# criteo/tf-yarn

Measured on AMD Instinct MI355X. Metric: examples/sec (whole node), Criteo wide-and-deep, higher is better.
Workload: dtype bf16; 1 GPU; model=wide_and_deep_criteo, global_batch=65536, per_gpu_batch=65536, dense_features=13, sparse_features=26, embedding_dim=16, table_rows_per_feature=1000000, parallelism=dp1, alltoall_mode=unprobed

## Files before the change

tf_yarn_amd/ops/__init__.py:

```python

from __future__ import annotations

import functools
import logging
import math
import os
from typing import NamedTuple, Optional, Tuple

import torch

logger = logging.getLogger(__name__)

try:
    from tf_yarn_amd.ops import _C
    HAVE_EXT = True
except ImportError as _e:
    _C = None
    HAVE_EXT = False
    _IMPORT_ERROR = _e


def _require_ext() -> None:
    if not HAVE_EXT:
        raise RuntimeError(
# ... 913 lines not shown
            batch, n_features * dim, device=table.device,
            dtype=torch.bfloat16 if out_bf16 else torch.float32)
        col_offset = 0
    if (out.dim() != 2 or out.shape[0] != batch or col_offset < 0
            or col_offset + n_features * dim > out.shape[1]):
        raise ValueError(
            f"the [{batch}, {n_features * dim}] block at column "
            f"{col_offset} does not fit out {tuple(out.shape)}")
    if _on_gpu(table, ids, out):
        _require_ext()
        bag_scale, flat = _C.emb_bag_fwd(table, ids, bag_offsets,
                                         n_features, offsets, weights,
                                         combiner, out, col_offset)
        return out, bag_scale, flat
    if _bounds_debug():
        _debug_check_bags(bag_offsets, ids.numel())
    bag_scale, flat = _emb_bag_fwd_ref(table, ids, bag_offsets, n_features,
                                       offsets, weights, combiner, out,
                                       col_offset)
    return out, bag_scale, flat


def emb_bag_bwd_rows(grad_out: torch.Tensor, bag_offsets: torch.Tensor,
                     bag_scale: torch.Tensor, dim: int, n_features: int, *,
                     weights: Optional[torch.Tensor] = None,
                     col_offset: int = 0,
                     nnz: Optional[int] = None) -> torch.Tensor:
    if nnz is None and weights is not None:
        nnz = int(weights.numel())
    batch = _check_bags(None, bag_offsets, n_features, weights, nnz)
    if bag_scale.numel() != batch * n_features:
        raise ValueError("bag_scale must have one entry per bag")
    if (grad_out.dim() != 2 or grad_out.shape[0] != batch or col_offset < 0
            or col_offset + n_features * dim > grad_out.shape[1]):
        raise ValueError(
            f"the [{batch}, {n_features * dim}] block at column "
            f"{col_offset} does not fit grad_out {tuple(grad_out.shape)}")
    if _on_gpu(grad_out, bag_offsets, bag_scale):
        _require_ext()
        if nnz is None:
            nnz = int(bag_offsets[-1].item())
        if grad_out.stride(1) != 1 or grad_out.stride(0) < grad_out.shape[1]:
            grad_out = grad_out.contiguous()
        return _C.emb_bag_bwd_rows(grad_out, bag_offsets, bag_scale, dim,
                                   n_features, nnz, weights, col_offset)
    _, lens = _bag_lengths(bag_offsets)
    n_bags = batch * n_features
    if _bounds_debug():
        _debug_check_bags(bag_offsets, int(lens.sum().item()))
    bag = torch.repeat_interleave(torch.arange(n_bags), lens)
    s = bag_scale[bag]
    if weights is not None:
        s = s * weights
    g = grad_out[:, col_offset:col_offset + n_features * dim] \
        .reshape(n_bags, dim)[bag]
    return (g.float() * s.unsqueeze(1)).to(grad_out.dtype)


class EmbeddingBagFn(torch.autograd.Function):

    @staticmethod
    def forward(ctx, table, ids, bag_offsets, n_features, offsets, weights,
                combiner, out_bf16, sink, dense, col_offset, wrap):
        dim = table.shape[1]
        batch = (bag_offsets.numel() - 1) // n_features
        out = None
        if dense is not None or col_offset:
            out = torch.empty(
                batch, col_offset + n_features * dim, device=table.device,
                dtype=torch.bfloat16 if out_bf16 else torch.float32)
            n_dense = 0
            if dense is not None:
                n_dense = dense.shape[1]
                out[:, :n_dense] = dense.to(out.dtype)
            out[:, n_dense:col_offset] = 0
        out, bag_scale, flat_ids = emb_bag_fwd(
            table.detach(), ids, bag_offsets, n_features, offsets=offsets,
            weights=weights, combiner=combiner, out=out,
            col_offset=col_offset, out_bf16=out_bf16)
        ctx.sink, ctx.wrap = sink, wrap
        ctx.dims = (dim, n_features, col_offset, ids.numel())
        ctx.weights = weights
        ctx.save_for_backward(bag_offsets, bag_scale, flat_ids)
        return out

    @staticmethod
    def backward(ctx, grad_out):
        bag_offsets, bag_scale, flat_ids = ctx.saved_tensors
        dim, n_features, col_offset, nnz = ctx.dims
        rows = emb_bag_bwd_rows(grad_out, bag_offsets, bag_scale, dim,
                                n_features, weights=ctx.weights,
                                col_offset=col_offset, nnz=nnz)
        ctx.sink.append(ctx.wrap((flat_ids, rows)))
        return (None,) * 12


def col_reduce_dot(x: torch.Tensor, dy: torch.Tensor) -> torch.Tensor:
    if _on_gpu(x, dy):
        _require_ext()
        return _C.col_reduce_dot(x.contiguous(), dy.contiguous())
    return (x.float() * dy.float().unsqueeze(1)).sum(dim=0)


def fused_head_grads_enabled() -> bool:
    return _env_switch_on("MIYARN_FUSED_HEAD_GRADS")


def col_reduce_dot_sum(x: torch.Tensor, dy: torch.Tensor,
                       out_dtype: torch.dtype = torch.float32):
    if _on_gpu(x, dy):
        _require_ext()
        if out_dtype in (torch.float32, torch.bfloat16):
            dw, db = _C.col_reduce_dot_sum(x.contiguous(), dy.contiguous(),
                                           out_dtype == torch.bfloat16)
            return dw, db
        dw, db = _C.col_reduce_dot_sum(x.contiguous(), dy.contiguous(),
                                       False)
        return dw.to(out_dtype), db.to(out_dtype)
    dw = (x.float() * dy.float().unsqueeze(1)).sum(dim=0)
    db = dy.float().sum().reshape(1)
    return dw.to(out_dtype), db.to(out_dtype)


def row_dot(x: torch.Tensor, w: torch.Tensor,
            bias: "torch.Tensor | None" = None) -> torch.Tensor:
    if _on_gpu(x, w) and x.size(1) % 4 == 0 and x.size(1) <= 512:
        _require_ext()
        return _C.row_dot(x.contiguous(), w.contiguous(), bias)
    y = x @ w
    return y if bias is None else y + bias


def gemm_bt(a: torch.Tensor, b: torch.Tensor,
            bias: "torch.Tensor | None" = None,
            relu: bool = False) -> torch.Tensor:
    if _on_gpu(a, b):
        _require_ext()
        return _C.gemm_bt(a.contiguous(), b.contiguous(), bias, relu)
    out = a.float() @ b.float().t()
    if bias is not None:
        out = out + bias.float()
    if relu:
        out = torch.relu(out)
    return out.to(a.dtype)


class ScalarHeadFn(torch.autograd.Function):

    @staticmethod
    def forward(ctx, x, weight, bias):
        ctx.save_for_backward(x, weight)
        if _on_gpu(x, weight) and x.size(1) % 4 == 0 \
                and x.size(1) <= 512 and bias.numel() == 1:
            _require_ext()
            return _C.row_dot(x.contiguous(), weight.contiguous(),
                              bias.reshape(1))
        return x @ weight + bias

    @staticmethod
    def backward(ctx, dy):
        x, weight = ctx.saved_tensors
        dy = dy.contiguous()
        dx = dw = db = None
        if ctx.needs_input_grad[0]:
            dx = dy.unsqueeze(1) * weight.unsqueeze(0)
        if ctx.needs_input_grad[1] and ctx.needs_input_grad[2] \
                and _on_gpu(x, dy) and x.dtype == dy.dtype \
                and fused_head_grads_enabled():
            dw, db = col_reduce_dot_sum(x, dy, weight.dtype)
            return dx, dw, db
        if ctx.needs_input_grad[1]:
            dw = col_reduce_dot(x, dy).to(weight.dtype)
        if ctx.needs_input_grad[2]:
            db = dy.sum().reshape(1).to(weight.dtype)
        return dx, dw, db


class BCEHeadFn(torch.autograd.Function):

    @staticmethod
    def forward(ctx, deep, wide, dhead, labels):
        if deep.is_cuda and HAVE_EXT and deep.dtype == torch.bfloat16 \
                and wide.dtype == torch.bfloat16 \
                and dhead.dtype == torch.bfloat16:
            loss, sig = _C.bce_head_fwd(
                deep.contiguous(), wide.contiguous(), dhead.contiguous(),
                labels.contiguous().float())
        else:
            z = (deep.float() + wide.float() + dhead.float())
            labels = labels.float()
            loss = torch.nn.functional.binary_cross_entropy_with_logits(
                z, labels, reduction="none")
            sig = torch.sigmoid(z).to(deep.dtype)
        ctx.save_for_backward(sig, labels)
        ctx.dtype = deep.dtype
        return loss

    @staticmethod
    def backward(ctx, g):
        sig, labels = ctx.saved_tensors
        if sig.is_cuda and HAVE_EXT and sig.dtype == torch.bfloat16:
            dl = _C.bce_head_bwd(sig, labels.contiguous().float(),
                                 g.contiguous().float())
        else:
            dl = ((sig.float() - labels.float()) * g.float()).to(ctx.dtype)
        return dl, dl, dl, None


def bce_head_loss(deep: torch.Tensor, wide: torch.Tensor,
                  dhead: torch.Tensor, labels: torch.Tensor) -> torch.Tensor:
    return BCEHeadFn.apply(deep, wide, dhead, labels).mean()


class BiasReLU(torch.autograd.Function):

    @staticmethod
    def forward(ctx, x, bias):
        y = bias_relu_fwd(x, bias)
        ctx.save_for_backward(y)
        return y

    @staticmethod
    def backward(ctx, dy):
        (y,) = ctx.saved_tensors
        if dy.is_cuda and HAVE_EXT and y.size(-1) % 4 == 0 \
                and y.size(-1) <= 8192:
            dx, dbias = _C.bias_relu_bwd_db(
                dy.contiguous(), y.contiguous(),
                dy.dtype == torch.bfloat16)
            return dx, dbias.to(dy.dtype)
        dx = bias_relu_bwd(dy.contiguous(), y)
        dims = tuple(range(dx.dim() - 1))
        dbias = dx.sum(dim=dims)
        return dx, dbias


def bias_relu(x: torch.Tensor, bias: torch.Tensor) -> torch.Tensor:
    return BiasReLU.apply(x, bias)


def _custom_wgrad_kernel(dz: torch.Tensor, x: torch.Tensor):
    if os.environ.get("MIYARN_WGRAD") == "lib":
        return None
    if not (dz.is_cuda and HAVE_EXT):
        return None
    if dz.dtype != torch.bfloat16 or x.dtype != torch.bfloat16:
        return None
    n, m = dz.size(1), x.size(1)
    if m % 8 != 0 or dz.size(0) % 64 != 0:
        return None
    if n % 256 == 0 and n * m > 256 * 512:
        return _C.wgrad_nt256
    if n % 128 == 0 and n * m <= 256 * 512:
        return _C.wgrad_nt128
    return None


def _fused_dgrad_shape_routed(k: int, n: int) -> bool:
    return (k, n) in _FUSED_DGRAD_SHAPES


_FUSED_DGRAD_SHAPES = frozenset({(256, 512), (512, 1024)})


def _custom_fwd_ok(x: torch.Tensor, weight: torch.Tensor,
                   bias: torch.Tensor) -> bool:
    if os.environ.get("MIYARN_FWD") != "custom":
        return False
    if not (x.is_cuda and HAVE_EXT):
        return False
    if x.dtype != torch.bfloat16 or weight.dtype != torch.bfloat16 \
            or bias.dtype != torch.bfloat16:
        return False
    if x.dim() != 2 or not x.is_contiguous() or not weight.is_contiguous():
        return False
    m, k = x.shape
    return m % 256 == 0 and k % 16 == 0 and weight.size(0) % 16 == 0


def _lt_fwd_ok(x, weight, bias) -> bool:
    if os.environ.get("MIYARN_LT_FWD", "1") in ("", "0"):
        return False
    return (x.is_cuda and HAVE_EXT and x.dim() == 2
            and x.dtype == torch.bfloat16
            and weight.dtype == torch.bfloat16
            and bias.dtype == torch.bfloat16
            and x.is_contiguous() and weight.is_contiguous())


def _linear_bias_relu_fwd(x: torch.Tensor, weight: torch.Tensor,
                          bias: torch.Tensor) -> torch.Tensor:
    if _custom_fwd_ok(x, weight, bias):
        return _C.gemm_bt(x, weight, bias, True)
    if _lt_fwd_ok(x, weight, bias):
        return _C.lt_linear(x, weight, bias.contiguous(), True)
    return bias_relu_fwd(x.matmul(weight.t()), bias)


def _linear_wgrad(dz: torch.Tensor, x: torch.Tensor,
                  weight: torch.Tensor) -> torch.Tensor:
    kernel = _custom_wgrad_kernel(dz, x)
    if kernel is None:
        return dz.t().matmul(x)
    dw = kernel(dz, x, 0, weight.dtype == torch.bfloat16)
    return dw if dw.dtype == weight.dtype else dw.to(weight.dtype)


class LinearBiasReLU(torch.autograd.Function):

    @staticmethod
    def forward(ctx, x, weight, bias):
        y = _linear_bias_relu_fwd(x, weight, bias)
        ctx.save_for_backward(x, weight, y)
        return y

    @staticmethod
    def backward(ctx, dy):
        x, weight, y = ctx.saved_tensors
        dy = dy.contiguous()
        if dy.is_cuda and HAVE_EXT and y.size(-1) % 4 == 0 \
                and y.size(-1) <= 8192:
            dz, dbias = _C.bias_relu_bwd_db(
                dy, y.contiguous(), dy.dtype == torch.bfloat16)
            if dbias.dtype != dy.dtype:
                dbias = dbias.to(dy.dtype)
        else:
            dz = bias_relu_bwd(dy, y)
            dbias = dz.sum(dim=tuple(range(dz.dim() - 1)))
        dx = dz.matmul(weight)
        return dx, _linear_wgrad(dz, x, weight), dbias


def linear_bias_relu(x: torch.Tensor, weight: torch.Tensor,
                     bias: torch.Tensor) -> torch.Tensor:
    return LinearBiasReLU.apply(x, weight, bias)



def fused_head_bwd_enabled() -> bool:
    return _env_switch_on("MIYARN_FUSED_HEAD_BWD")


def head_relu_bwd_db(dl: torch.Tensor, w_head: torch.Tensor,
                     y: torch.Tensor):
    if _on_gpu(dl, w_head, y) and HAVE_EXT and dl.dtype == y.dtype \
            and w_head.dtype == y.dtype and y.dim() == 2 \
            and y.size(1) % 4 == 0 and y.size(1) <= 8192:
        dz, dbias = _C.head_relu_bwd_db(
            dl.contiguous(), w_head.contiguous(), y.contiguous(),
            y.dtype == torch.bfloat16)
        return dz, dbias.to(y.dtype)
    if _on_gpu(dl, w_head, y):
        _require_ext()
    dz = bias_relu_bwd(dl.unsqueeze(1) * w_head.unsqueeze(0), y)
    return dz, dz.sum(dim=0)


def head_relu_bwd_grads(dl: torch.Tensor, w_head: torch.Tensor,
                        y: torch.Tensor):
    if _on_gpu(dl, w_head, y) and HAVE_EXT and dl.dtype == y.dtype \
            and w_head.dtype == y.dtype and y.dim() == 2 \
            and y.size(1) % 4 == 0 and y.size(1) <= 8192 \
            and y.dtype in (torch.float32, torch.bfloat16):
        dz, dbias, dw_head, db_head = _C.head_relu_bwd_grads(
            dl.contiguous(), w_head.contiguous(), y.contiguous(),
            y.dtype == torch.bfloat16)
        return dz, dbias, dw_head, db_head
    dw_head = col_reduce_dot(y, dl).to(w_head.dtype)
    db_head = dl.sum().reshape(1).to(w_head.dtype)
    dz, dbias = head_relu_bwd_db(dl, w_head, y)
    return dz, dbias, dw_head, db_head


class LinearBiasReLUHeadFn(torch.autograd.Function):

    @staticmethod
    def forward(ctx, x, weight, bias, w_head, b_head):
        y = _linear_bias_relu_fwd(x, weight, bias)
        ctx.save_for_backward(x, weight, y, w_head)
        if _on_gpu(y, w_head) and y.size(1) % 4 == 0 \
                and y.size(1) <= 512 and b_head.numel() == 1:
            _require_ext()
            return _C.row_dot(y.contiguous(), w_head.contiguous(),
                              b_head.reshape(1))
        return y @ w_head + b_head

    @staticmethod
    def backward(ctx, dl):
        x, weight, y, w_head = ctx.saved_tensors
        dl = dl.contiguous()
        dw_head = db_head = None
        if ctx.needs_input_grad[3] and ctx.needs_input_grad[4] \
                and _on_gpu(dl, y) and fused_head_grads_enabled():
            dz, dbias, dw_head, db_head = head_relu_bwd_grads(dl, w_head, y)
        else:
            if ctx.needs_input_grad[3]:
                dw_head = col_reduce_dot(y, dl).to(w_head.dtype)
            if ctx.needs_input_grad[4]:
                db_head = dl.sum().reshape(1).to(w_head.dtype)
            dz, dbias = head_relu_bwd_db(dl, w_head, y)
        dx = dz.matmul(weight)
        dw = _linear_wgrad(dz, x, weight)
        return dx, dw, dbias, dw_head, db_head


def linear_bias_relu_head(x: torch.Tensor, weight: torch.Tensor,
                          bias: torch.Tensor, w_head: torch.Tensor,
                          b_head: torch.Tensor) -> torch.Tensor:
    return LinearBiasReLUHeadFn.apply(x, weight, bias, w_head, b_head)



def fused_dgrad_enabled() -> bool:
    return _env_switch_on("MIYARN_FUSED_DGRAD")


def _dgrad_drelu_kernel_ok(dz_next: torch.Tensor, weight: torch.Tensor,
                           y: torch.Tensor) -> bool:
    if not (HAVE_EXT and dz_next.is_cuda and weight.is_cuda and y.is_cuda):
        return False
    if not (dz_next.dtype == weight.dtype == y.dtype == torch.bfloat16):
        return False
    if not (dz_next.dim() == 2 and weight.dim() == 2 and y.dim() == 2):
        return False
    m, k = dz_next.shape
    n = weight.shape[1]
    return (weight.shape[0] == k and tuple(y.shape) == (m, n) and m > 0
            and m % 256 == 0 and k % 16 == 0 and n % 16 == 0)


def dgrad_drelu(dz_next: torch.Tensor, weight: torch.Tensor,
                y: torch.Tensor):
    if _dgrad_drelu_kernel_ok(dz_next, weight, y):
        dz, dbias = _C.dgrad_drelu(dz_next.contiguous(),
                                   weight.contiguous(), y.contiguous(),
                                   True)
        return dz, dbias
    return _relu_bwd_db(dz_next.matmul(weight), y)


def _relu_bwd_db(dy: torch.Tensor, y: torch.Tensor):
    dy = dy.contiguous()
    if dy.is_cuda and HAVE_EXT and y.size(-1) % 4 == 0 \
            and y.size(-1) <= 8192:
        dz, dbias = _C.bias_relu_bwd_db(
            dy, y.contiguous(), dy.dtype == torch.bfloat16)
        if dbias.dtype != dy.dtype:
            dbias = dbias.to(dy.dtype)
        return dz, dbias
    dz = bias_relu_bwd(dy, y)
    return dz, dz.sum(dim=tuple(range(dz.dim() - 1)))


class MLPHeadFn(torch.autograd.Function):

    @staticmethod
    def forward(ctx, x, w_head, b_head, *wb):
        n = len(wb) // 2
        weights, biases = wb[:n], wb[n:]
        ys = []
        h = x
        for w, b in zip(weights, biases):
            h = _linear_bias_relu_fwd(h, w, b)
            ys.append(h)
        ctx.n_layers = n
        ctx.save_for_backward(x, w_head, *weights, *ys)
        if _on_gpu(h, w_head) and h.size(1) % 4 == 0 \
                and h.size(1) <= 512 and b_head.numel() == 1:
            _require_ext()
            return _C.row_dot(h.contiguous(), w_head.contiguous(),
                              b_head.reshape(1))
        return h @ w_head + b_head

    @staticmethod
    def backward(ctx, dl):
        n = ctx.n_layers
        saved = ctx.saved_tensors
        x, w_head = saved[0], saved[1]
        weights, ys = saved[2:2 + n], saved[2 + n:]
        dl = dl.contiguous()
        dw_head = db_head = None
        if ctx.needs_input_grad[1] and ctx.needs_input_grad[2] \
                and _on_gpu(dl, ys[-1]) and fused_head_grads_enabled():
            dz, dbias, dw_head, db_head = head_relu_bwd_grads(
                dl, w_head, ys[-1])
        else:
            if ctx.needs_input_grad[1]:
                dw_head = col_reduce_dot(ys[-1], dl).to(w_head.dtype)
            if ctx.needs_input_grad[2]:
                db_head = dl.sum().reshape(1).to(w_head.dtype)
            dz, dbias = head_relu_bwd_db(dl, w_head, ys[-1])
        dws = [None] * n
        dbs = [None] * n
        fused = fused_dgrad_enabled()
        for l in range(n - 1, 0, -1):
            w, y_below = weights[l], ys[l - 1]
            dws[l] = _linear_wgrad(dz, y_below, w)
            dbs[l] = dbias
            if fused and _fused_dgrad_shape_routed(*w.shape) \
                    and _dgrad_drelu_kernel_ok(dz, w, y_below):
                dz, dbias = dgrad_drelu(dz, w, y_below)
            else:
                dz, dbias = _relu_bwd_db(dz.matmul(w), y_below)
        dx = dz.matmul(weights[0]) if ctx.needs_input_grad[0] else None
        dws[0] = _linear_wgrad(dz, x, weights[0])
        dbs[0] = dbias
        return (dx, dw_head, db_head, *dws, *dbs)


def mlp_bias_relu_head(x: torch.Tensor, weights, biases,
                       w_head: torch.Tensor,
                       b_head: torch.Tensor) -> torch.Tensor:
    return MLPHeadFn.apply(x, w_head, b_head, *weights, *biases)


def mlp_head_routed(x: torch.Tensor, weights) -> bool:
    if not (fused_dgrad_enabled() and x.dim() == 2 and x.size(0) > 0
            and x.size(0) % 256 == 0):
        return False
    return any(_fused_dgrad_shape_routed(*w.shape) and w.shape[0] % 16 == 0
               and w.shape[1] % 16 == 0 for w in weights[1:])



EVAL_BUCKETS = 4096
EVAL_SLOTS = 256


class BinaryEvalState:

    def __init__(self, device=None):
        self.hist = torch.zeros(2, EVAL_BUCKETS, dtype=torch.int64,
                                device=device)
        self.counts = torch.zeros(4, dtype=torch.int64, device=device)
        self.sums = torch.zeros(EVAL_SLOTS, 2, dtype=torch.float64,
                                device=device)

    def tensors(self) -> Tuple[torch.Tensor, torch.Tensor, torch.Tensor]:
        return self.hist, self.counts, self.sums

    def zero_(self) -> "BinaryEvalState":
        for t in self.tensors():
            t.zero_()
        return self


def _binary_eval_update_ref(z: torch.Tensor, y: torch.Tensor,
                            state: BinaryEvalState) -> None:
    nan = torch.isnan(z) | torch.isnan(y)
    n_nan = int(nan.sum())
    z, y = z[~nan], y[~nan]
    pos = y >= 0.5
    hot = z > 0
    t = (z + 16.0) * 128.0
    k = torch.floor(t).clamp_(0.0, EVAL_BUCKETS - 1.0).to(torch.int64)
    state.hist[0] += torch.bincount(k[~pos], minlength=EVAL_BUCKETS)
    state.hist[1] += torch.bincount(k[pos], minlength=EVAL_BUCKETS)
    state.counts += torch.tensor(
        [z.numel(), n_nan, int((pos & hot).sum()), int((~pos & hot).sum())],
        dtype=torch.int64)
    loss = z.clamp_min(0.0) - z * y + torch.log1p(torch.exp(-z.abs()))
    sig = 1.0 / (1.0 + torch.exp(-z))
    state.sums[0, 0] += loss.double().sum()
    state.sums[0, 1] += sig.double().sum()


def binary_eval_update(logits: torch.Tensor, labels: torch.Tensor,
                       state: BinaryEvalState) -> None:
    z = logits.reshape(-1)
    y = labels.reshape(-1)
    if z.numel() != y.numel():
        raise ValueError(f"{z.numel()} logits but {y.numel()} labels")
    if y.dtype != torch.float32:
        y = y.float()
    if z.numel() == 0:
        return
    if _on_gpu(z, y, *state.tensors()):
        _require_ext()
        if z.dtype not in (torch.float32, torch.bfloat16):
            z = z.float()
        _C.binary_eval_update(z.contiguous(), y.contiguous(),
                              *state.tensors())
        return
    _binary_eval_update_ref(z.float(), y, state)
```

tf_yarn_amd/ops/csrc/bindings.cpp:

```cpp
#include <torch/extension.h>
#include <string>
#include <tuple>
#include <variant>
#include <vector>

void fused_sgd(torch::Tensor param, torch::Tensor grad,
               c10::optional<torch::Tensor> momentum_buf,
               c10::optional<torch::Tensor> param_bf16,
               double lr, double momentum, double dampening,
               double weight_decay, bool nesterov, bool first_step,
               double grad_scale);
void fused_sgd_mt(std::vector<torch::Tensor> params,
                  std::vector<torch::Tensor> grads,
                  std::vector<torch::Tensor> momentum_bufs,
                  std::vector<torch::Tensor> params_bf16,
                  double lr, double momentum, double dampening,
                  double weight_decay, bool nesterov, bool first_step,
                  double grad_scale);
void fused_adam(torch::Tensor param, torch::Tensor grad,
                torch::Tensor exp_avg, torch::Tensor exp_avg_sq,
                c10::optional<torch::Tensor> param_bf16,
                double lr, double beta1, double beta2, double eps,
                double weight_decay, bool adamw, int64_t step,
                double grad_scale);
void fused_adagrad(torch::Tensor param, torch::Tensor grad,
                   torch::Tensor state_sum, double lr, double eps,
                   double weight_decay, double grad_scale);
void fused_ftrl(torch::Tensor param, torch::Tensor grad,
                torch::Tensor accum, torch::Tensor linear, double lr,
                double l1, double l2, double grad_scale);
void fused_adadelta(torch::Tensor param, torch::Tensor grad,
                    torch::Tensor square_avg, torch::Tensor acc_delta,
                    double lr, double rho, double eps, double weight_decay,
                    double grad_scale);

torch::Tensor emb_fwd(torch::Tensor table, torch::Tensor ids, bool out_bf16);
void emb_bwd_sgd(torch::Tensor table, torch::Tensor ids, torch::Tensor grad,
                 double lr, double scale);
void emb_bwd_sgd_sorted(torch::Tensor table, torch::Tensor sorted_ids,
                        torch::Tensor grad, double lr, double scale);
void emb_bwd_dense(torch::Tensor grad_table, torch::Tensor ids,
                   torch::Tensor grad, double scale);
void emb_bwd_sgd_fused_wide_offs(torch::Tensor table,
                                 torch::Tensor wide_table, torch::Tensor ids,
                                 torch::Tensor grad, torch::Tensor gw,
                                 double lr, double scale,
                                 c10::optional<torch::Tensor> offsets);
bool emb_lookup_fused_ok(int64_t dim, int64_t n_features, int64_t n_dense,
                         int64_t col_offset, int64_t out_cols);
torch::Tensor emb_lookup_fused(torch::Tensor table, torch::Tensor wide_table,
                               torch::Tensor ids, torch::Tensor offsets,
                               c10::optional<torch::Tensor> dense,
                               torch::Tensor out, int64_t col_offset);

torch::Tensor emb_gather_sum(torch::Tensor table, torch::Tensor ids,
                             int64_t batch, bool out_bf16);
void emb_fwd_into(torch::Tensor table, torch::Tensor ids,
                  torch::Tensor out, int64_t col_offset);
void emb_scatter_sum(torch::Tensor table, torch::Tensor ids,
                     torch::Tensor grad, double alpha);

std::vector<torch::Tensor> emb_bag_fwd(
    torch::Tensor table, torch::Tensor ids, torch::Tensor bag_offsets,
    int64_t n_features, c10::optional<torch::Tensor> offsets,
    c10::optional<torch::Tensor> weights, const std::string& combiner,
    torch::Tensor out, int64_t col_offset);
torch::Tensor emb_bag_bwd_rows(torch::Tensor grad_out,
                               torch::Tensor bag_offsets,
                               torch::Tensor bag_scale, int64_t dim,
                               int64_t n_features, int64_t nnz,
                               c10::optional<torch::Tensor> weights,
                               int64_t col_offset);

using SparseSide9 = std::tuple<std::string, torch::Tensor,
                               std::vector<torch::Tensor>, torch::Tensor,
                               c10::optional<torch::Tensor>, double, double,
                               double, double>;
using SparseSide12 = std::tuple<std::string, torch::Tensor,
                                std::vector<torch::Tensor>, torch::Tensor,
                                c10::optional<torch::Tensor>, double, double,
                                double, double, double, double, int64_t>;
using SparseSide = std::variant<SparseSide9, SparseSide12>;
void emb_bwd_sparse(c10::optional<SparseSide> deep,
                    c10::optional<SparseSide> wide, torch::Tensor stamp,
                    torch::Tensor ids, int64_t epoch, double scale);
bool sparse_pair_fused_ok(const std::string& deep_rule,
                          const std::string& wide_rule, int64_t dim);
py::dict binned_layout();
std::vector<torch::Tensor> binned_permutation(torch::Tensor ids,
                                              int64_t n_rows,
                                              int64_t region_bits);
void emb_bwd_sgd_binned(torch::Tensor table, torch::Tensor ids,
                        torch::Tensor grad, double lr, double scale,
                        torch::Tensor order, torch::Tensor starts);
void emb_scatter_sum_binned(torch::Tensor table, torch::Tensor ids,
                            torch::Tensor grad, int64_t g_div,
                            double alpha, torch::Tensor order,
                            torch::Tensor starts);

torch::Tensor bias_relu_fwd(torch::Tensor x, torch::Tensor bias);
torch::Tensor bias_relu_bwd(torch::Tensor dy, torch::Tensor y);
std::vector<torch::Tensor> bias_relu_bwd_db(torch::Tensor dy,
                                            torch::Tensor y,
                                            bool dbias_bf16);
std::vector<torch::Tensor> head_relu_bwd_db(torch::Tensor dl,
                                            torch::Tensor w_head,
                                            torch::Tensor y,
                                            bool dbias_bf16);
std::vector<torch::Tensor> head_relu_bwd_grads(torch::Tensor dl,
                                               torch::Tensor w_head,
                                               torch::Tensor y,
                                               bool out_bf16);
torch::Tensor reduce_splitk(torch::Tensor part, bool out_bf16);
torch::Tensor reduce_tall(torch::Tensor part, bool out_bf16,
                          int64_t quad_lanes);

torch::Tensor lt_linear(torch::Tensor x, torch::Tensor w,
                        c10::optional<torch::Tensor> bias, bool relu);
torch::Tensor col_reduce_dot(torch::Tensor x, torch::Tensor dy);
std::vector<torch::Tensor> col_reduce_dot_sum(torch::Tensor x,
                                              torch::Tensor dy,
                                              bool out_bf16);
torch::Tensor row_dot(torch::Tensor x, torch::Tensor w,
                      c10::optional<torch::Tensor> bias);
std::vector<torch::Tensor> bce_head_fwd(torch::Tensor deep,
                                        torch::Tensor wide,
                                        torch::Tensor dhead,
                                        torch::Tensor labels);
torch::Tensor bce_head_bwd(torch::Tensor sig, torch::Tensor labels,
                           torch::Tensor g);

torch::Tensor wgrad_nt128(torch::Tensor dy, torch::Tensor x,
                          int64_t splitk, bool out_bf16);
torch::Tensor wgrad_nt256(torch::Tensor dy, torch::Tensor x,
                          int64_t splitk, bool out_bf16);
void convert_scaled(torch::Tensor src, torch::Tensor dst, double scale);

torch::Tensor gemm_bt(torch::Tensor a, torch::Tensor b,
                      c10::optional<torch::Tensor> bias, bool relu);

std::vector<torch::Tensor> dgrad_drelu(torch::Tensor dz_next, torch::Tensor w,
                                       torch::Tensor y, bool dbias_bf16);

void binary_eval_update(torch::Tensor logits, torch::Tensor labels,
                        torch::Tensor hist, torch::Tensor counts,
                        torch::Tensor sums);

PYBIND11_MODULE(TORCH_EXTENSION_NAME, m) {
  m.doc() = "tf_yarn_amd MI355X (gfx950) HIP kernels";
  m.def("fused_sgd", &fused_sgd, "Fused SGD(+momentum) step");
  m.def("fused_sgd_mt", &fused_sgd_mt,
        "Multi-tensor fused SGD (one launch per <=24 tensors)");
  m.def("fused_adam", &fused_adam, "Fused Adam/AdamW step");
  m.def("fused_adagrad", &fused_adagrad, "Fused Adagrad step");
  m.def("fused_adadelta", &fused_adadelta, "Fused Adadelta step");
  m.def("emb_fwd", &emb_fwd, "Fused multi-table embedding gather");
  m.def("emb_bwd_sgd", &emb_bwd_sgd,
        "Fused sparse embedding grad scatter + SGD update");
  m.def("emb_bwd_sgd_sorted", &emb_bwd_sgd_sorted,
        "Atomic-free segmented scatter+SGD over SORTED ids");
  m.def("emb_bwd_sgd_fused_wide", &emb_bwd_sgd_fused_wide_offs,
        "Fused deep scatter+SGD + wide scalar scatter (shared ids; with "
        "offsets, raw [batch, features] ids)",
        py::arg("table"), py::arg("wide_table"), py::arg("ids"),
        py::arg("grad"), py::arg("gw"), py::arg("lr"), py::arg("scale"),
        py::arg("offsets") = py::none());
  m.def("emb_lookup_fused_ok", &emb_lookup_fused_ok,
        "Whether emb_lookup_fused covers (dim, features, n_dense, "
        "col_offset, out_cols)");
  m.def("emb_lookup_fused", &emb_lookup_fused,
        "Offset add + deep gather into a slice + wide gather-sum + dense/"
        "pad columns in one kernel (returns the wide sums)",
        py::arg("table"), py::arg("wide_table"), py::arg("ids"),
        py::arg("offsets"), py::arg("dense"), py::arg("out"),
        py::arg("col_offset"));
  m.def("emb_bag_fwd", &emb_bag_fwd,
        "Pooled multi-hot lookup from CSR bags into a column slice of out; "
        "returns (bag_scale, flat_ids)",
        py::arg("table"), py::arg("ids"), py::arg("bag_offsets"),
        py::arg("n_features"), py::arg("offsets"), py::arg("weights"),
        py::arg("combiner"), py::arg("out"), py::arg("col_offset"));
  m.def("emb_bag_bwd_rows", &emb_bag_bwd_rows,
        "Pooled gradients -> per-entry update rows [nnz, dim]",
        py::arg("grad_out"), py::arg("bag_offsets"), py::arg("bag_scale"),
        py::arg("dim"), py::arg("n_features"), py::arg("nnz"),
        py::arg("weights"), py::arg("col_offset"));
  m.def("emb_bwd_dense", &emb_bwd_dense,
        "Sparse embedding grad scatter into dense grad table");
  m.def("emb_bwd_sparse", &emb_bwd_sparse,
        "Stateful sparse update (adagrad, ftrl, rowwise_adagrad, lazy_adam) "
        "of a deep "
        "side, a wide side or both from shared ids: atomic accumulate + "
        "once-per-row claim/apply; sides without gradients run the apply "
        "alone on their accumulators",
        py::arg("deep"), py::arg("wide"), py::arg("stamp"), py::arg("ids"),
        py::arg("epoch"), py::arg("scale"));
  m.def("sparse_pair_fused_ok", &sparse_pair_fused_ok,
        "Whether emb_bwd_sparse has a fused deep+wide kernel for (deep rule, "
        "wide rule, deep dim)");
  m.def("fused_ftrl", &fused_ftrl, "Fused dense FTRL-proximal step");
  m.def("bias_relu_fwd", &bias_relu_fwd, "Fused bias+ReLU forward");
  m.def("bias_relu_bwd", &bias_relu_bwd, "Fused ReLU backward");
  m.def("lt_linear", &lt_linear,
        "hipBLASLt linear with fused bias(+ReLU) epilogue",
        py::arg("x"), py::arg("w"), py::arg("bias") = py::none(),
        py::arg("relu") = false);
  m.def("reduce_splitk", &reduce_splitk,
        "Split-K partial reduction with fused output cast",
        py::arg("part"), py::arg("out_bf16") = false);
  m.def("reduce_tall", &reduce_tall,
        "reduce_splitk's tall-slab kernel with 1 or 4 quad lanes per block",
        py::arg("part"), py::arg("out_bf16") = false,
        py::arg("quad_lanes") = 1);
  m.def("wgrad_nt128", &wgrad_nt128,
        "Split-K MFMA weight gradient dW = dy^T @ x (bf16 in), 128x128 tiles",
        py::arg("dy"), py::arg("x"), py::arg("splitk"),
        py::arg("out_bf16") = false);
  m.def("wgrad_nt256", &wgrad_nt256,
        "Split-K MFMA weight gradient dW = dy^T @ x (bf16 in), 256x256 tiles",
        py::arg("dy"), py::arg("x"), py::arg("splitk"),
        py::arg("out_bf16") = false);
  m.def("col_reduce_dot", &col_reduce_dot,
        "dw[m] = sum_b dy[b] * x[b,m] (single-logit head wgrad)");
  m.def("col_reduce_dot_sum", &col_reduce_dot_sum,
        "col_reduce_dot plus db = sum_b dy[b] from the same pass "
        "(returns [dw, db])",
        py::arg("x"), py::arg("dy"), py::arg("out_bf16") = false);
  m.def("row_dot", &row_dot,
        "y[b] = x[b].w + bias (single-logit head forward GEMV)");
  m.def("bce_head_fwd", &bce_head_fwd,
        "Fused 3-part logit sum + stable BCEWithLogits (loss, sigmoid)");
  m.def("bce_head_bwd", &bce_head_bwd,
        "dlogit = (sigmoid - label) * upstream grad");
  m.def("bias_relu_bwd_db", &bias_relu_bwd_db,
        "Fused ReLU backward + dbias reduction (returns [dx, dbias])",
        py::arg("dy"), py::arg("y"), py::arg("dbias_bf16") = false);
  m.def("head_relu_bwd_db", &head_relu_bwd_db,
        "ReLU backward + dbias of the layer under a single-logit head, from "
        "dl and w_head (no outer product; returns [dz, dbias])",
        py::arg("dl"), py::arg("w_head"), py::arg("y"),
        py::arg("dbias_bf16") = false);
  m.def("head_relu_bwd_grads", &head_relu_bwd_grads,
        "head_relu_bwd_db plus the head's own dw and db from the same pass "
        "(returns [dz, dbias, dw_head, db_head])",
        py::arg("dl"), py::arg("w_head"), py::arg("y"),
        py::arg("out_bf16") = false);
  m.def("emb_fwd_into", &emb_fwd_into,
        "Embedding gather into a slice of a larger 2D buffer");
  m.def("emb_gather_sum", &emb_gather_sum,
        "Wide-part gather-sum: out[b] = sum_f table[ids[b,f]]");
  m.def("binned_layout", &binned_layout,
        "Layout constants of the binned scatter (hash capacities, probe "
        "limit, hash threshold, launch shapes)");
  m.def("binned_permutation", &binned_permutation,
        "Region-binned permutation of sparse update indices");
  m.def("emb_bwd_sgd_binned", &emb_bwd_sgd_binned,
        "Binned LDS-dedup scatter+SGD (deep tables, dim=16)");
  m.def("emb_scatter_sum_binned", &emb_scatter_sum_binned,
        "Binned LDS-dedup scatter-add (scalar wide tables)");
  m.def("emb_scatter_sum", &emb_scatter_sum,
        "Wide-part scatter: table[ids[b,f]] += alpha * g[b]");
  m.def("convert_scaled", &convert_scaled, "Scaled bf16<->fp32 convert");
  m.def("gemm_bt", &gemm_bt,
        "C = A @ B^T (both K-major bf16) with fused bias+ReLU epilogue");
  m.def("dgrad_drelu", &dgrad_drelu,
        "Hidden-layer dgrad dz_next @ w with the ReLU backward of the layer "
        "below and its dbias in the epilogue (returns [dz, dbias])",
        py::arg("dz_next"), py::arg("w"), py::arg("y"),
        py::arg("dbias_bf16") = false);
  m.def("binary_eval_update", &binary_eval_update,
        "Fold a batch of (logit, label) into the streaming binary eval "
        "state: score histogram [2, 4096], counts (n_valid, n_nan, tp, fp), "
        "per-slot fp64 (loss, sigmoid) sums [256, 2]",
        py::arg("logits"), py::arg("labels"), py::arg("hist"),
        py::arg("counts"), py::arg("sums"));
}
```

tf_yarn_amd/ops/csrc/mfma_tile.h:

```cpp
#pragma once

#include "common.h"

typedef __attribute__((ext_vector_type(8))) __bf16 mfma_bf16x8;
typedef __attribute__((ext_vector_type(4))) float mfma_f32x4;

__device__ __forceinline__ int lds_off(int n, int k) {
  int byte = n * 128 + k * 2;
  const int s = ((n ^ (n >> 3)) & 7) | (((n >> 6) & 1) << 3);
  return byte ^ (s << 4);
}

__device__ __forceinline__ int lds_off_linear(int r, int k) {
  int byte = r * 128 + k * 2;
  return byte ^ (((r ^ (r >> 3)) & 7) << 4);
}
```

tf_yarn_amd/ops/csrc/wgrad.hip:

```cpp

#include <torch/extension.h>
#include <c10/hip/HIPStream.h>
#include "mfma_tile.h"

torch::Tensor reduce_splitk(torch::Tensor part, bool out_bf16);

namespace {

#define WG_BK 64

union U16x4 {
  unsigned short u[4];
  unsigned long long ll;
};

template <int TILE>
__global__ __launch_bounds__(2 * TILE)
void wgrad_kernel(const unsigned short* __restrict__ dy,
                  const unsigned short* __restrict__ x,
                  float* __restrict__ part,
                  int64_t B, int N, int M, int64_t chunk) {
  constexpr int FN = 4;
  constexpr int FM = TILE / 32;
  constexpr int SC = TILE / 8;

  const int tiles_m = (M + TILE - 1) / TILE;
  const int tile_n = blockIdx.y / tiles_m;
  const int tile_m = blockIdx.y - tile_n * tiles_m;
  const int n0 = tile_n * TILE;
  const int m0 = tile_m * TILE;
  const int64_t k_begin = (int64_t)blockIdx.x * chunk;
  const int64_t k_end = min(B, k_begin + chunk);

  __shared__ __attribute__((aligned(16))) unsigned char
      lds_raw[2 * TILE * 128];
  unsigned char* dyT = lds_raw;
  unsigned char* xT = lds_raw + TILE * 128;

  const int tid = threadIdx.x;
  const int lane = tid & 63;
  const int wave = tid >> 6;
  const int wn = (wave >> 1) * 64;
  const int wm = (wave & 1) * (TILE / 2);

  const int st_kg = (tid / SC) * 4;
  const int st_c = (tid % SC) * 8;

  mfma_f32x4 acc[FN][FM];
#pragma unroll
  for (int i = 0; i < FN; ++i)
#pragma unroll
    for (int j = 0; j < FM; ++j) acc[i][j] = {0.f, 0.f, 0.f, 0.f};

  const int a_row = lane & 15;
  const int a_k = (lane >> 4) * 8;
  const bool m_edge = (m0 + TILE) > M;
  const bool in0 = !m_edge || (m0 + st_c + 4) <= M;
  const bool in1 = !m_edge || (m0 + st_c + 8) <= M;

  bf16x4 rdy[4][2], rx[4][2];

  auto load_step = [&](int64_t k0) {
#pragma unroll
    for (int rr = 0; rr < 4; ++rr) {
      const unsigned short* src =
          dy + (k0 + st_kg + rr) * (int64_t)N + n0 + st_c;
      rdy[rr][0] = reinterpret_cast<const bf16x4*>(src)[0];
      rdy[rr][1] = reinterpret_cast<const bf16x4*>(src)[1];
      const unsigned short* srcx =
          x + (k0 + st_kg + rr) * (int64_t)M + m0 + st_c;
      rx[rr][0] = bf16x4{0, 0, 0, 0};
      rx[rr][1] = bf16x4{0, 0, 0, 0};
      if (in0) rx[rr][0] = reinterpret_cast<const bf16x4*>(srcx)[0];
      if (in1) rx[rr][1] = reinterpret_cast<const bf16x4*>(srcx)[1];
    }
  };

  auto write_step = [&] {
#pragma unroll
    for (int h = 0; h < 2; ++h)
#pragma unroll
      for (int j = 0; j < 4; ++j) {
        U16x4 p{{rdy[0][h][j], rdy[1][h][j], rdy[2][h][j], rdy[3][h][j]}};
        *reinterpret_cast<unsigned long long*>(
            dyT + lds_off(st_c + h * 4 + j, st_kg)) = p.ll;
        U16x4 q{{rx[0][h][j], rx[1][h][j], rx[2][h][j], rx[3][h][j]}};
        *reinterpret_cast<unsigned long long*>(
            xT + lds_off(st_c + h * 4 + j, st_kg)) = q.ll;
      }
  };

  load_step(k_begin);
  for (int64_t k0 = k_begin; k0 < k_end; k0 += WG_BK) {
    write_step();
    __syncthreads();
    if (k0 + WG_BK < k_end)
      load_step(k0 + WG_BK);
#pragma unroll
    for (int kh = 0; kh < 2; ++kh) {
      mfma_bf16x8 a[FN], b[FM];
#pragma unroll
      for (int i = 0; i < FN; ++i)
        a[i] = *reinterpret_cast<const mfma_bf16x8*>(
            dyT + lds_off(wn + i * 16 + a_row, kh * 32 + a_k));
#pragma unroll
      for (int j = 0; j < FM; ++j)
        b[j] = *reinterpret_cast<const mfma_bf16x8*>(
            xT + lds_off(wm + j * 16 + a_row, kh * 32 + a_k));
#pragma unroll
      for (int i = 0; i < FN; ++i)
#pragma unroll
        for (int j = 0; j < FM; ++j)
          acc[i][j] = __builtin_amdgcn_mfma_f32_16x16x32_bf16(
              a[i], b[j], acc[i][j], 0, 0, 0);
    }
    __syncthreads();
  }

  float* out = part + (int64_t)blockIdx.x * N * M;
  const int c_col = lane & 15;
  const int c_row = (lane >> 4) * 4;
#pragma unroll
  for (int i = 0; i < FN; ++i)
#pragma unroll
    for (int j = 0; j < FM; ++j) {
      const int col = m0 + wm + j * 16 + c_col;
      if (col >= M) continue;
#pragma unroll
      for (int r = 0; r < 4; ++r) {
        const int row = n0 + wn + i * 16 + c_row + r;
        out[(int64_t)row * M + col] = acc[i][j][r];
      }
    }
}

template <int TILE>
torch::Tensor wgrad_launch(torch::Tensor dy, torch::Tensor x,
                           int64_t splitk, bool out_bf16) {
  TORCH_CHECK(dy.is_cuda() && dy.is_contiguous() && dy.dim() == 2 &&
              dy.scalar_type() == torch::kBFloat16,
              "dy must be [B, N] bf16 contiguous");
  TORCH_CHECK(x.is_cuda() && x.is_contiguous() && x.dim() == 2 &&
              x.scalar_type() == torch::kBFloat16,
              "x must be [B, M] bf16 contiguous");
  const int64_t B = dy.size(0);
  const int N = static_cast<int>(dy.size(1));
  const int M = static_cast<int>(x.size(1));
  TORCH_CHECK(x.size(0) == B, "batch mismatch");
  TORCH_CHECK(N % TILE == 0 && M % 8 == 0 && B % WG_BK == 0,
              "wgrad_nt", TILE, " needs N % ", TILE,
              " == 0, M % 8 == 0, B % 64 == 0");
  const int tiles = (N / TILE) * ((M + TILE - 1) / TILE);
  constexpr int budget = TILE == 256 ? 256 : 512;
  if (splitk <= 0)
    splitk = std::min<int64_t>(
        32, std::max<int64_t>(1, budget / std::max(1, tiles)));
  int64_t chunk = ((B + splitk - 1) / splitk + WG_BK - 1) / WG_BK * WG_BK;
  splitk = (B + chunk - 1) / chunk;
  auto part = torch::empty({splitk, N, M},
                           dy.options().dtype(torch::kFloat32));
  auto stream = c10::hip::getCurrentHIPStream().stream();
  dim3 grid(splitk, tiles);
  hipLaunchKernelGGL(wgrad_kernel<TILE>, grid, dim3(2 * TILE), 0, stream,
                     reinterpret_cast<unsigned short*>(dy.data_ptr()),
                     reinterpret_cast<unsigned short*>(x.data_ptr()),
                     part.data_ptr<float>(), B, N, M, chunk);
  return reduce_splitk(part, out_bf16);
}

}

torch::Tensor wgrad_nt128(torch::Tensor dy, torch::Tensor x,
                          int64_t splitk, bool out_bf16) {
  return wgrad_launch<128>(dy, x, splitk, out_bf16);
}

torch::Tensor wgrad_nt256(torch::Tensor dy, torch::Tensor x,
                          int64_t splitk, bool out_bf16) {
  return wgrad_launch<256>(dy, x, splitk, out_bf16);
}
```

Before: 59.03 million examples/s.

## Stage wgrad tiles via LDS-DMA with double buffering and transposed LDS reads

Adds a wgrad kernel variant that loads dy and x tiles straight from global memory into LDS with global_load_lds_dwordx4, double-buffers the stages, and reads MFMA operands with ds_read_tr16 transposed loads under a new swizzle. The goal is to drop the register-staged transpose and the extra VGPR traffic, and to overlap the next k-step load with compute. This variant becomes the default for both tile sizes, and an env var can select the old path. It doubles LDS usage, which may lower occupancy, and it relies on inline asm that changes m0. Edge columns are clamped rather than zero-filled, which may be wrong when M is not a multiple of the tile.

```diff
diff --git a/tf_yarn_amd/ops/__init__.py b/tf_yarn_amd/ops/__init__.py
--- a/tf_yarn_amd/ops/__init__.py
+++ b/tf_yarn_amd/ops/__init__.py
@@ -1239,7 +1239,8 @@
     kernel = _custom_wgrad_kernel(dz, x)
     if kernel is None:
         return dz.t().matmul(x)
-    dw = kernel(dz, x, 0, weight.dtype == torch.bfloat16)
+    regstage = True if os.environ.get("MIYARN_WGRAD") == "regstage" else None
+    dw = kernel(dz, x, 0, weight.dtype == torch.bfloat16, regstage)
     return dw if dw.dtype == weight.dtype else dw.to(weight.dtype)
 
 
diff --git a/tf_yarn_amd/ops/csrc/bindings.cpp b/tf_yarn_amd/ops/csrc/bindings.cpp
--- a/tf_yarn_amd/ops/csrc/bindings.cpp
+++ b/tf_yarn_amd/ops/csrc/bindings.cpp
@@ -131,9 +131,12 @@
                            torch::Tensor g);
 
 torch::Tensor wgrad_nt128(torch::Tensor dy, torch::Tensor x,
-                          int64_t splitk, bool out_bf16);
+                          int64_t splitk, bool out_bf16,
+                          c10::optional<bool> regstage);
 torch::Tensor wgrad_nt256(torch::Tensor dy, torch::Tensor x,
-                          int64_t splitk, bool out_bf16);
+                          int64_t splitk, bool out_bf16,
+                          c10::optional<bool> regstage);
+py::dict wgrad_glds_layout();
 void convert_scaled(torch::Tensor src, torch::Tensor dst, double scale);
 
 torch::Tensor gemm_bt(torch::Tensor a, torch::Tensor b,
@@ -213,13 +216,19 @@
         py::arg("part"), py::arg("out_bf16") = false,
         py::arg("quad_lanes") = 1);
   m.def("wgrad_nt128", &wgrad_nt128,
-        "Split-K MFMA weight gradient dW = dy^T @ x (bf16 in), 128x128 tiles",
+        "Split-K MFMA weight gradient dW = dy^T @ x (bf16 in), 128x128 tiles; "
+        "regstage: True = register-staged k-loop, False = LDS-DMA staging "
+        "with transposed LDS reads, None = this tile's measured default",
         py::arg("dy"), py::arg("x"), py::arg("splitk"),
-        py::arg("out_bf16") = false);
+        py::arg("out_bf16") = false, py::arg("regstage") = py::none());
   m.def("wgrad_nt256", &wgrad_nt256,
-        "Split-K MFMA weight gradient dW = dy^T @ x (bf16 in), 256x256 tiles",
+        "Split-K MFMA weight gradient dW = dy^T @ x (bf16 in), 256x256 tiles; "
+        "regstage: True = register-staged k-loop, False = LDS-DMA staging "
+        "with transposed LDS reads, None = this tile's measured default",
         py::arg("dy"), py::arg("x"), py::arg("splitk"),
-        py::arg("out_bf16") = false);
+        py::arg("out_bf16") = false, py::arg("regstage") = py::none());
+  m.def("wgrad_glds_layout", &wgrad_glds_layout,
+        "Constants and image table of the wgrad kernels' LDS-DMA staging");
   m.def("col_reduce_dot", &col_reduce_dot,
         "dw[m] = sum_b dy[b] * x[b,m] (single-logit head wgrad)");
   m.def("col_reduce_dot_sum", &col_reduce_dot_sum,
diff --git a/tf_yarn_amd/ops/csrc/mfma_tile.h b/tf_yarn_amd/ops/csrc/mfma_tile.h
--- a/tf_yarn_amd/ops/csrc/mfma_tile.h
+++ b/tf_yarn_amd/ops/csrc/mfma_tile.h
@@ -15,3 +15,10 @@
   int byte = r * 128 + k * 2;
   return byte ^ (((r ^ (r >> 3)) & 7) << 4);
 }
+
+__host__ __device__ constexpr int lds_swz_tr(int row) {
+  return ((row & 3) << 2) | ((row >> 2) & 3);
+}
+__host__ __device__ constexpr int lds_off_tr(int row, int ch) {
+  return 256 * row + 16 * (ch ^ lds_swz_tr(row));
+}
diff --git a/tf_yarn_amd/ops/csrc/wgrad.hip b/tf_yarn_amd/ops/csrc/wgrad.hip
--- a/tf_yarn_amd/ops/csrc/wgrad.hip
+++ b/tf_yarn_amd/ops/csrc/wgrad.hip
@@ -14,7 +14,15 @@
   unsigned long long ll;
 };
 
-template <int TILE>
+constexpr int WG_IMG_COLS = 128;
+constexpr int WG_IMG_BYTES = WG_BK * 2 * WG_IMG_COLS;
+constexpr int WG_FILL_ROWS = 4;
+constexpr int WG_FILLS_PER_WAVE = 8;
+
+typedef __attribute__((ext_vector_type(4))) __bf16 mfma_bf16x4;
+#define WG_LDS_AS __attribute__((address_space(3)))
+
+template <int TILE, bool GLDS>
 __global__ __launch_bounds__(2 * TILE)
 void wgrad_kernel(const unsigned short* __restrict__ dy,
                   const unsigned short* __restrict__ x,
@@ -33,9 +41,7 @@
   const int64_t k_end = min(B, k_begin + chunk);
 
   __shared__ __attribute__((aligned(16))) unsigned char
-      lds_raw[2 * TILE * 128];
-  unsigned char* dyT = lds_raw;
-  unsigned char* xT = lds_raw + TILE * 128;
+      lds_raw[(GLDS ? 4 : 2) * TILE * 128];
 
   const int tid = threadIdx.x;
   const int lane = tid & 63;
@@ -43,78 +49,182 @@
   const int wn = (wave >> 1) * 64;
   const int wm = (wave & 1) * (TILE / 2);
 
-  const int st_kg = (tid / SC) * 4;
-  const int st_c = (tid % SC) * 8;
-
   mfma_f32x4 acc[FN][FM];
 #pragma unroll
   for (int i = 0; i < FN; ++i)
 #pragma unroll
     for (int j = 0; j < FM; ++j) acc[i][j] = {0.f, 0.f, 0.f, 0.f};
 
-  const int a_row = lane & 15;
-  const int a_k = (lane >> 4) * 8;
-  const bool m_edge = (m0 + TILE) > M;
-  const bool in0 = !m_edge || (m0 + st_c + 4) <= M;
-  const bool in1 = !m_edge || (m0 + st_c + 8) <= M;
-
-  bf16x4 rdy[4][2], rx[4][2];
-
-  auto load_step = [&](int64_t k0) {
-#pragma unroll
-    for (int rr = 0; rr < 4; ++rr) {
-      const unsigned short* src =
-          dy + (k0 + st_kg + rr) * (int64_t)N + n0 + st_c;
-      rdy[rr][0] = reinterpret_cast<const bf16x4*>(src)[0];
-      rdy[rr][1] = reinterpret_cast<const bf16x4*>(src)[1];
-      const unsigned short* srcx =
-          x + (k0 + st_kg + rr) * (int64_t)M + m0 + st_c;
-      rx[rr][0] = bf16x4{0, 0, 0, 0};
-      rx[rr][1] = bf16x4{0, 0, 0, 0};
-      if (in0) rx[rr][0] = reinterpret_cast<const bf16x4*>(srcx)[0];
-      if (in1) rx[rr][1] = reinterpret_cast<const bf16x4*>(srcx)[1];
-    }
-  };
-
-  auto write_step = [&] {
-#pragma unroll
-    for (int h = 0; h < 2; ++h)
-#pragma unroll
-      for (int j = 0; j < 4; ++j) {
-        U16x4 p{{rdy[0][h][j], rdy[1][h][j], rdy[2][h][j], rdy[3][h][j]}};
-        *reinterpret_cast<unsigned long long*>(
-            dyT + lds_off(st_c + h * 4 + j, st_kg)) = p.ll;
-        U16x4 q{{rx[0][h][j], rx[1][h][j], rx[2][h][j], rx[3][h][j]}};
-        *reinterpret_cast<unsigned long long*>(
-            xT + lds_off(st_c + h * 4 + j, st_kg)) = q.ll;
-      }
-  };
-
-  load_step(k_begin);
-  for (int64_t k0 = k_begin; k0 < k_end; k0 += WG_BK) {
-    write_step();
-    __syncthreads();
-    if (k0 + WG_BK < k_end)
-      load_step(k0 + WG_BK);
-#pragma unroll
-    for (int kh = 0; kh < 2; ++kh) {
-      mfma_bf16x8 a[FN], b[FM];
-#pragma unroll
-      for (int i = 0; i < FN; ++i)
-        a[i] = *reinterpret_cast<const mfma_bf16x8*>(
-            dyT + lds_off(wn + i * 16 + a_row, kh * 32 + a_k));
-#pragma unroll
-      for (int j = 0; j < FM; ++j)
-        b[j] = *reinterpret_cast<const mfma_bf16x8*>(
-            xT + lds_off(wm + j * 16 + a_row, kh * 32 + a_k));
-#pragma unroll
-      for (int i = 0; i < FN; ++i)
+  if constexpr (GLDS) {
+    constexpr int NI = TILE / WG_IMG_COLS;
+    constexpr int OPB = NI * WG_IMG_BYTES;
+    constexpr int BUFB = 2 * OPB;
+    constexpr int WPO = TILE / 64;
+
+    const int uw = __builtin_amdgcn_readfirstlane(wave);
+    const int f_op = uw / WPO;
+    const int f_grp = (uw % WPO) * WG_FILLS_PER_WAVE;
+    const int f_img = f_grp / 16;
+    const int f_r0 = (f_grp % 16) * WG_FILL_ROWS;
+    const unsigned short* f_ptr = f_op ? x : dy;
+    const int f_ld = f_op ? M : N;
+    const int f_cmax = f_ld / 8 - 1;
+    const int f_c0 = (f_op ? m0 : n0) / 8 + f_img * 16;
+    const int f_row = f_r0 + (lane >> 4);
+    const unsigned short* f_src[4];
+#pragma unroll
+    for (int t = 0; t < 4; ++t) {
+      const int row = f_row + WG_FILL_ROWS * t;
+      const int ch = min(f_c0 + ((lane & 15) ^ lds_swz_tr(row)), f_cmax);
+      f_src[t] = f_ptr + (int64_t)row * f_ld + ch * 8;
+    }
+    const unsigned f_dst =
+        (unsigned)(uintptr_t)(WG_LDS_AS unsigned char*)lds_raw +
+        f_op * OPB + f_img * WG_IMG_BYTES + f_r0 * 256;
+
+    auto stage = [&](int64_t k0, int bufoff) {
+      const int64_t koff = k0 * f_ld;
+#pragma unroll
+      for (int t = 0; t < WG_FILLS_PER_WAVE; ++t) {
+        const unsigned short* src =
+            f_src[t & 3] + koff + (int64_t)(t >> 2) * 16 * f_ld;
+        const unsigned dst = f_dst + bufoff + t * WG_FILL_ROWS * 256;
+        unsigned keep;
+        asm volatile(
+            "s_mov_b32 %0, m0\n\ts_mov_b32 m0, %2\n\ts_nop 0\n\t"
+            "global_load_lds_dwordx4 %1, off\n\ts_mov_b32 m0, %0"
+            : "=&s"(keep)
+            : "v"(src), "s"(dst)
+            : "memory");
+      }
+    };
+
+    const int t_q = (lane >> 2) & 3, t_p = lane & 3, t_g = lane >> 4;
+    int a_base[2], b_base[2];
+#pragma unroll
+    for (int h = 0; h < 2; ++h) {
+      const int row = 8 * t_g + 4 * h + t_q;
+      const int o = lds_off_tr(row, t_p >> 1) + 8 * (t_p & 1);
+      a_base[h] = (o ^ (((wn & 127) >> 4) << 5)) + (wn >> 7) * WG_IMG_BYTES;
+      b_base[h] = (o ^ (((wm & 127) >> 4) << 5)) + (wm >> 7) * WG_IMG_BYTES +
+                  OPB;
+    }
+
+    auto tr_read = [&](int off) {
+      return __builtin_amdgcn_ds_read_tr16_b64_v4bf16(
+          (WG_LDS_AS mfma_bf16x4*)(lds_raw + off));
+    };
+
+    auto compute = [&](int bufoff) {
+#pragma unroll
+      for (int kh = 0; kh < 2; ++kh) {
+        mfma_bf16x8 a[FN], b[FM];
+        const int ko = bufoff + kh * 32 * 256;
+#pragma unroll
+        for (int i = 0; i < FN; ++i)
+          a[i] = __builtin_shufflevector(
+              tr_read((a_base[0] ^ (i << 5)) + ko),
+              tr_read((a_base[1] ^ (i << 5)) + ko), 0, 1, 2, 3, 4, 5, 6, 7);
 #pragma unroll
         for (int j = 0; j < FM; ++j)
-          acc[i][j] = __builtin_amdgcn_mfma_f32_16x16x32_bf16(
-              a[i], b[j], acc[i][j], 0, 0, 0);
-    }
-    __syncthreads();
+          b[j] = __builtin_shufflevector(
+              tr_read((b_base[0] ^ (j << 5)) + ko),
+              tr_read((b_base[1] ^ (j << 5)) + ko), 0, 1, 2, 3, 4, 5, 6, 7);
+#pragma unroll
+        for (int i = 0; i < FN; ++i)
+#pragma unroll
+          for (int j = 0; j < FM; ++j)
+            acc[i][j] = __builtin_amdgcn_mfma_f32_16x16x32_bf16(
+                a[i], b[j], acc[i][j], 0, 0, 0);
+      }
+    };
+
+    auto publish = [] {
+      asm volatile("s_waitcnt vmcnt(0)" ::: "memory");
+      __syncthreads();
+    };
+
+    int cur = 0;
+    stage(k_begin, cur);
+    publish();
+    for (int64_t k0 = k_begin + WG_BK; k0 < k_end; k0 += WG_BK) {
+      stage(k0, cur ^ BUFB);
+      compute(cur);
+      publish();
+      cur ^= BUFB;
+    }
+    compute(cur);
+  } else {
+    unsigned char* dyT = lds_raw;
+    unsigned char* xT = lds_raw + TILE * 128;
+
+    const int st_kg = (tid / SC) * 4;
+    const int st_c = (tid % SC) * 8;
+
+    const int a_row = lane & 15;
+    const int a_k = (lane >> 4) * 8;
+    const bool m_edge = (m0 + TILE) > M;
+    const bool in0 = !m_edge || (m0 + st_c + 4) <= M;
+    const bool in1 = !m_edge || (m0 + st_c + 8) <= M;
+
+    bf16x4 rdy[4][2], rx[4][2];
+
+    auto load_step = [&](int64_t k0) {
+#pragma unroll
+      for (int rr = 0; rr < 4; ++rr) {
+        const unsigned short* src =
+            dy + (k0 + st_kg + rr) * (int64_t)N + n0 + st_c;
+        rdy[rr][0] = reinterpret_cast<const bf16x4*>(src)[0];
+        rdy[rr][1] = reinterpret_cast<const bf16x4*>(src)[1];
+        const unsigned short* srcx =
+            x + (k0 + st_kg + rr) * (int64_t)M + m0 + st_c;
+        rx[rr][0] = bf16x4{0, 0, 0, 0};
+        rx[rr][1] = bf16x4{0, 0, 0, 0};
+        if (in0) rx[rr][0] = reinterpret_cast<const bf16x4*>(srcx)[0];
+        if (in1) rx[rr][1] = reinterpret_cast<const bf16x4*>(srcx)[1];
+      }
+    };
+
+    auto write_step = [&] {
+#pragma unroll
+      for (int h = 0; h < 2; ++h)
+#pragma unroll
+        for (int j = 0; j < 4; ++j) {
+          U16x4 p{{rdy[0][h][j], rdy[1][h][j], rdy[2][h][j], rdy[3][h][j]}};
+          *reinterpret_cast<unsigned long long*>(
+              dyT + lds_off(st_c + h * 4 + j, st_kg)) = p.ll;
+          U16x4 q{{rx[0][h][j], rx[1][h][j], rx[2][h][j], rx[3][h][j]}};
+          *reinterpret_cast<unsigned long long*>(
+              xT + lds_off(st_c + h * 4 + j, st_kg)) = q.ll;
+        }
+    };
+
+    load_step(k_begin);
+    for (int64_t k0 = k_begin; k0 < k_end; k0 += WG_BK) {
+      write_step();
+      __syncthreads();
+      if (k0 + WG_BK < k_end)
+        load_step(k0 + WG_BK);
+#pragma unroll
+      for (int kh = 0; kh < 2; ++kh) {
+        mfma_bf16x8 a[FN], b[FM];
+#pragma unroll
+        for (int i = 0; i < FN; ++i)
+          a[i] = *reinterpret_cast<const mfma_bf16x8*>(
+              dyT + lds_off(wn + i * 16 + a_row, kh * 32 + a_k));
+#pragma unroll
+        for (int j = 0; j < FM; ++j)
+          b[j] = *reinterpret_cast<const mfma_bf16x8*>(
+              xT + lds_off(wm + j * 16 + a_row, kh * 32 + a_k));
+#pragma unroll
+        for (int i = 0; i < FN; ++i)
+#pragma unroll
+          for (int j = 0; j < FM; ++j)
+            acc[i][j] = __builtin_amdgcn_mfma_f32_16x16x32_bf16(
+                a[i], b[j], acc[i][j], 0, 0, 0);
+      }
+      __syncthreads();
+    }
   }
 
   float* out = part + (int64_t)blockIdx.x * N * M;
@@ -135,8 +245,12 @@
 }
 
 template <int TILE>
+constexpr bool kGldsDefault = TILE == 128 || TILE == 256;
+
+template <int TILE>
 torch::Tensor wgrad_launch(torch::Tensor dy, torch::Tensor x,
-                           int64_t splitk, bool out_bf16) {
+                           int64_t splitk, bool out_bf16,
+                           c10::optional<bool> regstage) {
   TORCH_CHECK(dy.is_cuda() && dy.is_contiguous() && dy.dim() == 2 &&
               dy.scalar_type() == torch::kBFloat16,
               "dy must be [B, N] bf16 contiguous");
@@ -161,7 +275,9 @@
                            dy.options().dtype(torch::kFloat32));
   auto stream = c10::hip::getCurrentHIPStream().stream();
   dim3 grid(splitk, tiles);
-  hipLaunchKernelGGL(wgrad_kernel<TILE>, grid, dim3(2 * TILE), 0, stream,
+  const bool glds = regstage.has_value() ? !*regstage : kGldsDefault<TILE>;
+  auto kernel = glds ? wgrad_kernel<TILE, true> : wgrad_kernel<TILE, false>;
+  hipLaunchKernelGGL(kernel, grid, dim3(2 * TILE), 0, stream,
                      reinterpret_cast<unsigned short*>(dy.data_ptr()),
                      reinterpret_cast<unsigned short*>(x.data_ptr()),
                      part.data_ptr<float>(), B, N, M, chunk);
@@ -171,11 +287,32 @@
 }
 
 torch::Tensor wgrad_nt128(torch::Tensor dy, torch::Tensor x,
-                          int64_t splitk, bool out_bf16) {
-  return wgrad_launch<128>(dy, x, splitk, out_bf16);
+                          int64_t splitk, bool out_bf16,
+                          c10::optional<bool> regstage) {
+  return wgrad_launch<128>(dy, x, splitk, out_bf16, regstage);
 }
 
 torch::Tensor wgrad_nt256(torch::Tensor dy, torch::Tensor x,
-                          int64_t splitk, bool out_bf16) {
-  return wgrad_launch<256>(dy, x, splitk, out_bf16);
-}
+                          int64_t splitk, bool out_bf16,
+                          c10::optional<bool> regstage) {
+  return wgrad_launch<256>(dy, x, splitk, out_bf16, regstage);
+}
+
+py::dict wgrad_glds_layout() {
+  py::dict d;
+  d["bk"] = WG_BK;
+  d["img_cols"] = WG_IMG_COLS;
+  d["img_bytes"] = WG_IMG_BYTES;
+  d["fill_rows"] = WG_FILL_ROWS;
+  d["fills_per_wave"] = WG_FILLS_PER_WAVE;
+  d["buffers"] = 2;
+  py::list off;
+  for (int row = 0; row < WG_BK; ++row)
+    for (int ch = 0; ch < 16; ++ch) off.append(lds_off_tr(row, ch));
+  d["off"] = off;
+  py::dict def;
+  def[py::int_(128)] = kGldsDefault<128>;
+  def[py::int_(256)] = kGldsDefault<256>;
+  d["glds_default"] = def;
+  return d;
+}
```

After: 61.43 million examples/s (median of 6 runs). 4.1% higher.
